# AnneLouisedb/dlwp-benchmark

Measured on AMD Instinct MI355X. Metric: rollout cell-steps/s, higher is better.
Workload: dtype f32 (f16x3: products from two-part f16 splits, 22-bit operands, fp32 accumulate)

## Files before the change

### dlwp_benchmark_amd/csrc/fno_device.hpp

```cpp
#pragma once

#include "common.hpp"

namespace dlwp {
namespace fno {

constexpr int kC = 32;
constexpr int kTrStride = 68;

struct ChanSeg {
  const float* ptr;
  long long bstride;
  int nchan;
  int pad;
};
struct ChanTable {
  ChanSeg seg[4];
};

__device__ __forceinline__ const float* chan_ptr(const ChanTable& t, int c, int b, int HW) {
  const float* p = nullptr;
  int base = 0;
#pragma unroll
  for (int i = 0; i < 4; ++i) {
    const int n = t.seg[i].nchan;
    if (c >= base && c < base + n)
      p = t.seg[i].ptr + (long long)b * t.seg[i].bstride + (long long)(c - base) * HW;
    base += n;
  }
  return p;
}

__device__ __forceinline__ void wave_lds_fence() {
  __builtin_amdgcn_fence(__ATOMIC_ACQ_REL, "wavefront");
  __builtin_amdgcn_wave_barrier();
}

template <int NT, int KP>
__device__ __forceinline__ void fwd_dft_accumulate(const float* s_tr, const float* __restrict__ tt,
                                                   int w0, int lane, f32x4 (&yacc)[NT][KP / 16]) {
  const int j = lane & 15, g = lane >> 4;
#pragma unroll
  for (int s = 0; s < 16; ++s) {
    float bt[KP / 16];
#pragma unroll
    for (int kt = 0; kt < KP / 16; ++kt) bt[kt] = tt[(long long)(w0 + 4 * s + g) * KP + kt * 16 + j];
#pragma unroll
    for (int ct = 0; ct < NT; ++ct) {
      const float a = s_tr[(16 * ct + j) * kTrStride + 4 * s + g];
#pragma unroll
      for (int kt = 0; kt < KP / 16; ++kt) yacc[ct][kt] = mfma16x16x4(a, bt[kt], yacc[ct][kt]);
    }
  }
}

template <int NT, int KP>
__device__ __forceinline__ void store_y(float* __restrict__ ybuf, long long row, int nchan, int lane,
                                        const f32x4 (&yacc)[NT][KP / 16], int c0 = 0) {
  const int j = lane & 15, g = lane >> 4;
#pragma unroll
  for (int ct = 0; ct < NT; ++ct)
#pragma unroll
    for (int kt = 0; kt < KP / 16; ++kt)
      *reinterpret_cast<f32x4*>(ybuf + (row * KP + kt * 16 + j) * nchan + c0 + 16 * ct + 4 * g) = yacc[ct][kt];
}

struct MlpParams {
  ChanTable x;
  int hid;
  int cout;
  const float* w1p;
  const float* b1;
  const float* w2p;
  const float* b2;
  float* out;
  long long out_bstride;
  const float* resid;
  long long resid_bstride;
  float* ybuf;
  const float* tt;
  int B, H, W;
};

template <int CIN_STEPS, bool F16 = false>
__device__ __forceinline__ void lift_segment(const f32x4 (&xs)[CIN_STEPS], const float* s_w1, const float* s_b1,
                                             const u32x4* s_w2, int npair, int lane, const f32x4 (&bias2)[2],
                                             f32x4 (&acc2)[2][4], int ns = CIN_STEPS, bool cin1 = false, float f16_up = 1.f,
                                             float f16_down = 1.f) {
  const int g = lane >> 4;
  f32x4 xbc = {0.f, 0.f, 0.f, 0.f};
  if (cin1) {
#pragma unroll
    for (int q = 0; q < 4; ++q) {
      float v = xs[0][q];
      v += __shfl_xor(v, 16);
      v += __shfl_xor(v, 32);
      xbc[q] = v;
    }
  }
#pragma unroll
  for (int ot = 0; ot < 2; ++ot)
#pragma unroll
    for (int q = 0; q < 4; ++q) acc2[ot][q] = F16 ? bias2[ot] * f16_up : bias2[ot];

  u32x4 bg0[2][3], bg1[2][3];
  f32x4 a1[2][2];
  u32x4 wa[2][3];
  const int nunit = npair * 2;
  auto unit_valu_fc1 = [&](int u, auto qpc) {
    constexpr int qp = decltype(qpc)::value;
#pragma unroll
    for (int tt = 0; tt < 2; ++tt) {
      const int t = 2 * u + tt;
      const f32x4 bb = *reinterpret_cast<const f32x4*>(s_b1 + 16 * t + 4 * g);
      if (cin1) {
        const f32x4 wv = *reinterpret_cast<const f32x4*>(s_w1 + t * 64 + 4 * g);
#pragma unroll
        for (int qq = 0; qq < 2; ++qq)
#pragma unroll
          for (int r = 0; r < 4; ++r) a1[tt][qq][r] = __builtin_fmaf(wv[r], xbc[2 * qp + qq], bb[r]);
        continue;
      }
#pragma unroll
      for (int qq = 0; qq < 2; ++qq) a1[tt][qq] = bb;
#pragma unroll
      for (int s = 0; s < CIN_STEPS; ++s) {
        if (s >= ns) break;
        const float a = s_w1[(t * ns + s) * 64 + lane];
#pragma unroll
        for (int qq = 0; qq < 2; ++qq) a1[tt][qq] = mfma16x16x4(a, xs[s][2 * qp + qq], a1[tt][qq]);
      }
    }
  };
  auto unit_split = [&](u32x4(&bg)[2][3]) {
#pragma unroll
    for (int qq = 0; qq < 2; ++qq)
#pragma unroll
      for (int i = 0; i < 4; ++i) {
        unsigned hh, mm, ll;
        split_pair_x<F16>(a1[i / 2][qq][2 * (i % 2)], a1[i / 2][qq][2 * (i % 2) + 1], hh, mm, ll);
        bg[qq][0][i] = hh;
        bg[qq][1][i] = mm;
        bg[qq][2][i] = ll;
      }
  };
  auto load_wa = [&](int u) {
#pragma unroll
    for (int ot = 0; ot < 2; ++ot)
#pragma unroll
      for (int pp = 0; pp < 3; ++pp) wa[ot][pp] = s_w2[((u * 3 + pp) * 2 + ot) * 64 + lane];
  };
  auto unit_mfma = [&](const u32x4(&bg)[2][3], auto qpc, auto slotc) {
    constexpr int qp = decltype(qpc)::value, slot = decltype(slotc)::value;
    if constexpr (F16) {
      constexpr int PA[3] = {1, 0, 2}, PB[3] = {0, 1, 0};
#pragma unroll
      for (int ot = 0; ot < 2; ++ot)
#pragma unroll
        for (int qq = 0; qq < 2; ++qq)
          acc2[ot][2 * qp + qq] = mfma16x16x32_f16(wa[ot][PA[slot]], bg[qq][PB[slot]], acc2[ot][2 * qp + qq]);
    } else {
    constexpr int PA[6] = {2, 0, 1, 1, 0, 0}, PB[6] = {0, 2, 1, 0, 1, 0};
#pragma unroll
    for (int term = 2 * slot; term < 2 * slot + 2; ++term)
#pragma unroll
      for (int ot = 0; ot < 2; ++ot)
#pragma unroll
        for (int qq = 0; qq < 2; ++qq)
          acc2[ot][2 * qp + qq] = mfma16x16x32_bf16(wa[ot][PA[term]], bg[qq][PB[term]], acc2[ot][2 * qp + qq]);
    }
  };
  using I0 = std::integral_constant<int, 0>;
  using I1 = std::integral_constant<int, 1>;
  using I2 = std::integral_constant<int, 2>;
  auto trip = [&](int u_m, int u_v, const u32x4(&bgm)[2][3], u32x4(&bgv)[2][3], auto qm, auto qv) {
    load_wa(u_m);
    unit_valu_fc1(u_v, qv);
    unit_mfma(bgm, qm, I0{});
    gelu_erf8(a1[0][0], a1[0][1]);
    __builtin_amdgcn_sched_barrier(0);
    unit_mfma(bgm, qm, I1{});
    gelu_erf8(a1[1][0], a1[1][1]);
    __builtin_amdgcn_sched_barrier(0);
    unit_mfma(bgm, qm, I2{});
    unit_split(bgv);
    __builtin_amdgcn_sched_barrier(0);
  };
  unit_valu_fc1(0, I0{});
  gelu_erf8(a1[0][0], a1[0][1]);
  gelu_erf8(a1[1][0], a1[1][1]);
  unit_split(bg0);
  for (int u = 0; u < npair; ++u) {
    trip(u, u, bg0, bg1, I0{}, I1{});
    if (u + 1 < npair) trip(u, u + 1, bg1, bg0, I1{}, I0{});
  }
  load_wa(npair - 1);
  unit_mfma(bg1, I1{}, I0{});
  unit_mfma(bg1, I1{}, I1{});
  unit_mfma(bg1, I1{}, I2{});
  (void)nunit;
  if constexpr (F16) {
#pragma unroll
    for (int ot = 0; ot < 2; ++ot)
#pragma unroll
      for (int q = 0; q < 4; ++q) acc2[ot][q] *= f16_down;
  }

}

constexpr int kLiftTabRange = 32, kLiftTabLog2 = 4;
constexpr int kLiftTabCoefs = 6;
constexpr int kLiftTabStride = kLiftTabCoefs * kC;

__host__ __device__ __forceinline__ int lift_tab_locate(float x, int n_side, float scale, float& v) {
  const float a = fabsf(x) * scale;
  const float fl = floorf(a);
  v = a - fl;
  int k = (int)fl;
  k = k < 0 ? 0 : (k > n_side - 1 ? n_side - 1 : k);
  return x < 0.f ? n_side - 1 - k : n_side + k;
}

__device__ __forceinline__ void lift_from_table(const float* __restrict__ tab, const f32x4& xbc, int g, f32x4 (&vv)[2][4]) {
#pragma unroll
  for (int qp = 0; qp < 2; ++qp) {
    f32x4 c[2][kLiftTabCoefs][2];
    float v[2];
#pragma unroll
    for (int qq = 0; qq < 2; ++qq) {
      const int idx = lift_tab_locate(xbc[2 * qp + qq], kLiftTabRange << kLiftTabLog2, (float)(1 << kLiftTabLog2), v[qq]);
      const f32x4* src = reinterpret_cast<const f32x4*>(tab + (size_t)idx * kLiftTabStride + 4 * g);
#pragma unroll
      for (int k = kLiftTabCoefs - 1; k >= 0; --k) {
        c[qq][k][0] = src[k * (kC / 4)];
        c[qq][k][1] = src[k * (kC / 4) + 4];
      }
    }
#pragma unroll
    for (int qq = 0; qq < 2; ++qq)
#pragma unroll
      for (int ot = 0; ot < 2; ++ot) {
        f32x4 acc = c[qq][kLiftTabCoefs - 1][ot];
#pragma unroll
        for (int k = kLiftTabCoefs - 2; k >= 0; --k)
#pragma unroll
          for (int r = 0; r < 4; ++r) acc[r] = __builtin_fmaf(acc[r], v[qq], c[qq][k][ot][r]);
#pragma unroll
        for (int r = 0; r < 4; ++r) vv[ot][r][2 * qp + qq] = acc[r];
      }
  }
}

template <int CO, bool F16 = false>
__device__ __forceinline__ void proj_segment(const u32x4 (&bx)[4][3], const u32x4* s_w1, const float* s_b1,
                                             const float* s_w2, int ntile, int lane, float (&po)[CO][4], float f16_down = 1.f) {
  const int g = lane >> 4;
#pragma unroll
  for (int co = 0; co < CO; ++co)
#pragma unroll
    for (int q = 0; q < 4; ++q) po[co][q] = 0.f;
  auto fc1 = [&](int t, f32x4(&a1)[4]) {
    const f32x4 bb = *reinterpret_cast<const f32x4*>(s_b1 + 16 * t + 4 * g);
    u32x4 wa[3];
#pragma unroll
    for (int pp = 0; pp < 3; ++pp) wa[pp] = s_w1[(t * 3 + pp) * 64 + lane];
#pragma unroll
    for (int q = 0; q < 4; ++q) a1[q] = mfma_x<F16>(wa, bx[q], bb);
  };
  f32x4 a_cur[4], a_nxt[4], g_prev[4], g_new[4];
  fc1(0, a_cur);
  fc1(ntile > 1 ? 1 : 0, a_nxt);
#pragma unroll
  for (int q = 0; q < 4; ++q) g_prev[q] = F16 ? a_cur[q] * f16_down : a_cur[q];
  gelu_erf8(g_prev[0], g_prev[1]);
  gelu_erf8(g_prev[2], g_prev[3]);
#pragma unroll
  for (int q = 0; q < 4; ++q) a_cur[q] = a_nxt[q];
  u32x4 wa[3], wa_n[3];
  f32x4 w2v[CO], w2v_n[CO], bb, bb_n;
  {
    const int tn = ntile > 2 ? 2 : ntile - 1;
#pragma unroll
    for (int pp = 0; pp < 3; ++pp) wa[pp] = s_w1[(tn * 3 + pp) * 64 + lane];
#pragma unroll
    for (int co = 0; co < CO; ++co) w2v[co] = *reinterpret_cast<const f32x4*>(s_w2 + co * 16 + 4 * g);
    bb = *reinterpret_cast<const f32x4*>(s_b1 + 16 * tn + 4 * g);
  }
  for (int t = 1; t < ntile; ++t) {
    {
      const int tn2 = (t + 2 < ntile) ? t + 2 : ntile - 1;
#pragma unroll
      for (int pp = 0; pp < 3; ++pp) wa_n[pp] = s_w1[(tn2 * 3 + pp) * 64 + lane];
#pragma unroll
      for (int co = 0; co < CO; ++co) w2v_n[co] = *reinterpret_cast<const f32x4*>(s_w2 + (t * CO + co) * 16 + 4 * g);
      bb_n = *reinterpret_cast<const f32x4*>(s_b1 + 16 * tn2 + 4 * g);
    }
#pragma unroll
    for (int i = 0; i < 2; ++i) {
      a_nxt[2 * i] = mfma_x<F16>(wa, bx[2 * i], bb);
      a_nxt[2 * i + 1] = mfma_x<F16>(wa, bx[2 * i + 1], bb);
      g_new[2 * i] = F16 ? a_cur[2 * i] * f16_down : a_cur[2 * i];
      g_new[2 * i + 1] = F16 ? a_cur[2 * i + 1] * f16_down : a_cur[2 * i + 1];
      gelu_erf8(g_new[2 * i], g_new[2 * i + 1]);
#pragma unroll
      for (int co = 0; co < CO; ++co)
#pragma unroll
        for (int qq = 2 * i; qq < 2 * i + 2; ++qq)
#pragma unroll
          for (int r = 0; r < 4; ++r) po[co][qq] = fmaf(w2v[co][r], g_prev[qq][r], po[co][qq]);
      __builtin_amdgcn_sched_barrier(0);
    }
#pragma unroll
    for (int q = 0; q < 4; ++q) {
      g_prev[q] = g_new[q];
      a_cur[q] = a_nxt[q];
    }
#pragma unroll
    for (int pp = 0; pp < 3; ++pp) wa[pp] = wa_n[pp];
#pragma unroll
    for (int co = 0; co < CO; ++co) w2v[co] = w2v_n[co];
    bb = bb_n;
  }
  {
    const int t = ntile - 1;
#pragma unroll
    for (int co = 0; co < CO; ++co) {
      const f32x4 w2 = *reinterpret_cast<const f32x4*>(s_w2 + (t * CO + co) * 16 + 4 * g);
#pragma unroll
      for (int q = 0; q < 4; ++q)
#pragma unroll
        for (int r = 0; r < 4; ++r) po[co][q] = fmaf(w2[r], g_prev[q][r], po[co][q]);
    }
  }
}

struct LayerParams {
  const float* x;
  float* y;
  const float* wsp;
  const u32x4* wsb;
  const float* bias;
  const float* zbuf;
  const float* t;
  const float* tt;
  float* ybuf;
  int B, H, W;
  int stagger;
};

__device__ __forceinline__ float2 cfma(float2 a, float2 b, float2 c) {
  return float2{fmaf(a.x, b.x, fmaf(-a.y, b.y, c.x)), fmaf(a.x, b.y, fmaf(a.y, b.x, c.y))};
}

constexpr int kTrunkF16Shift = 3;
constexpr float kTrunkF16Up = 16384.0f, kTrunkF16Down = 1.0f / 16384.0f;

}
}
```

Baseline: 2.363 billion.

## Restructure projection pipeline into half-tile stages with register-light prefetch

Rewrites the projection segment's software pipeline so MFMA for the next tile, GELU for the current half-tile, and the FC2 FMAs for the previous half-tile are interleaved at half-tile granularity. The separate next-iteration copies of weights and activations are dropped in favour of single buffers reloaded in place, which lowers register pressure. Inline asm register pins keep each accumulator chain grouped. The added scheduling barriers fix the instruction order, but reloading buffers in place could expose LDS latency.

```diff
diff --git a/dlwp_benchmark_amd/csrc/fno_device.hpp b/dlwp_benchmark_amd/csrc/fno_device.hpp
--- a/dlwp_benchmark_amd/csrc/fno_device.hpp
+++ b/dlwp_benchmark_amd/csrc/fno_device.hpp
@@ -255,83 +255,68 @@
 __device__ __forceinline__ void proj_segment(const u32x4 (&bx)[4][3], const u32x4* s_w1, const float* s_b1,
                                              const float* s_w2, int ntile, int lane, float (&po)[CO][4], float f16_down = 1.f) {
   const int g = lane >> 4;
+  u32x4 wa[3];
+  f32x4 bb, w2v[CO];
+  auto load_l1 = [&](int t) {
+#pragma unroll
+    for (int pp = 0; pp < 3; ++pp) wa[pp] = s_w1[(t * 3 + pp) * 64 + lane];
+    bb = *reinterpret_cast<const f32x4*>(s_b1 + 16 * t + 4 * g);
+  };
+  auto load_l2 = [&](int t) {
+#pragma unroll
+    for (int co = 0; co < CO; ++co) w2v[co] = *reinterpret_cast<const f32x4*>(s_w2 + (t * CO + co) * 16 + 4 * g);
+  };
+  auto down = [&](const f32x4& a) -> f32x4 { return F16 ? a * f16_down : a; };
 #pragma unroll
   for (int co = 0; co < CO; ++co)
 #pragma unroll
     for (int q = 0; q < 4; ++q) po[co][q] = 0.f;
-  auto fc1 = [&](int t, f32x4(&a1)[4]) {
-    const f32x4 bb = *reinterpret_cast<const f32x4*>(s_b1 + 16 * t + 4 * g);
-    u32x4 wa[3];
-#pragma unroll
-    for (int pp = 0; pp < 3; ++pp) wa[pp] = s_w1[(t * 3 + pp) * 64 + lane];
-#pragma unroll
-    for (int q = 0; q < 4; ++q) a1[q] = mfma_x<F16>(wa, bx[q], bb);
-  };
-  f32x4 a_cur[4], a_nxt[4], g_prev[4], g_new[4];
-  fc1(0, a_cur);
-  fc1(ntile > 1 ? 1 : 0, a_nxt);
-#pragma unroll
-  for (int q = 0; q < 4; ++q) g_prev[q] = F16 ? a_cur[q] * f16_down : a_cur[q];
-  gelu_erf8(g_prev[0], g_prev[1]);
-  gelu_erf8(g_prev[2], g_prev[3]);
-#pragma unroll
-  for (int q = 0; q < 4; ++q) a_cur[q] = a_nxt[q];
-  u32x4 wa[3], wa_n[3];
-  f32x4 w2v[CO], w2v_n[CO], bb, bb_n;
-  {
-    const int tn = ntile > 2 ? 2 : ntile - 1;
-#pragma unroll
-    for (int pp = 0; pp < 3; ++pp) wa[pp] = s_w1[(tn * 3 + pp) * 64 + lane];
-#pragma unroll
-    for (int co = 0; co < CO; ++co) w2v[co] = *reinterpret_cast<const f32x4*>(s_w2 + co * 16 + 4 * g);
-    bb = *reinterpret_cast<const f32x4*>(s_b1 + 16 * tn + 4 * g);
-  }
+  auto fma2 = [&](int q0, const f32x4(&gg)[2]) {
+#pragma unroll
+    for (int co = 0; co < CO; ++co)
+#pragma unroll
+      for (int qq = 0; qq < 2; ++qq) {
+        float acc = po[co][q0 + qq];
+        asm("" : "+v"(acc));
+#pragma unroll
+        for (int r = 0; r < 4; ++r) acc = fmaf(w2v[co][r], gg[qq][r], acc);
+        asm("" : "+v"(acc));
+        po[co][q0 + qq] = acc;
+      }
+  };
+  f32x4 a[4], ga[2], gb[2];
+  load_l1(0);
+#pragma unroll
+  for (int q = 0; q < 4; ++q) a[q] = mfma_x<F16>(wa, bx[q], bb);
+  load_l1(ntile > 1 ? 1 : 0);
+  load_l2(0);
+  ga[0] = down(a[0]); ga[1] = down(a[1]);
+  gb[0] = down(a[2]); gb[1] = down(a[3]);
+#pragma unroll
+  for (int q = 0; q < 4; ++q) a[q] = mfma_x<F16>(wa, bx[q], bb);
+  load_l1(ntile > 2 ? 2 : ntile - 1);
+  gelu_erf8(ga[0], ga[1]);
+  gelu_erf8(gb[0], gb[1]);
+  fma2(0, ga);
   for (int t = 1; t < ntile; ++t) {
-    {
-      const int tn2 = (t + 2 < ntile) ? t + 2 : ntile - 1;
-#pragma unroll
-      for (int pp = 0; pp < 3; ++pp) wa_n[pp] = s_w1[(tn2 * 3 + pp) * 64 + lane];
-#pragma unroll
-      for (int co = 0; co < CO; ++co) w2v_n[co] = *reinterpret_cast<const f32x4*>(s_w2 + (t * CO + co) * 16 + 4 * g);
-      bb_n = *reinterpret_cast<const f32x4*>(s_b1 + 16 * tn2 + 4 * g);
-    }
-#pragma unroll
-    for (int i = 0; i < 2; ++i) {
-      a_nxt[2 * i] = mfma_x<F16>(wa, bx[2 * i], bb);
-      a_nxt[2 * i + 1] = mfma_x<F16>(wa, bx[2 * i + 1], bb);
-      g_new[2 * i] = F16 ? a_cur[2 * i] * f16_down : a_cur[2 * i];
-      g_new[2 * i + 1] = F16 ? a_cur[2 * i + 1] * f16_down : a_cur[2 * i + 1];
-      gelu_erf8(g_new[2 * i], g_new[2 * i + 1]);
-#pragma unroll
-      for (int co = 0; co < CO; ++co)
-#pragma unroll
-        for (int qq = 2 * i; qq < 2 * i + 2; ++qq)
-#pragma unroll
-          for (int r = 0; r < 4; ++r) po[co][qq] = fmaf(w2v[co][r], g_prev[qq][r], po[co][qq]);
-      __builtin_amdgcn_sched_barrier(0);
-    }
-#pragma unroll
-    for (int q = 0; q < 4; ++q) {
-      g_prev[q] = g_new[q];
-      a_cur[q] = a_nxt[q];
-    }
-#pragma unroll
-    for (int pp = 0; pp < 3; ++pp) wa[pp] = wa_n[pp];
-#pragma unroll
-    for (int co = 0; co < CO; ++co) w2v[co] = w2v_n[co];
-    bb = bb_n;
-  }
-  {
-    const int t = ntile - 1;
-#pragma unroll
-    for (int co = 0; co < CO; ++co) {
-      const f32x4 w2 = *reinterpret_cast<const f32x4*>(s_w2 + (t * CO + co) * 16 + 4 * g);
-#pragma unroll
-      for (int q = 0; q < 4; ++q)
-#pragma unroll
-        for (int r = 0; r < 4; ++r) po[co][q] = fmaf(w2[r], g_prev[q][r], po[co][q]);
-    }
-  }
+    ga[0] = down(a[0]); ga[1] = down(a[1]);
+    __builtin_amdgcn_sched_barrier(0);
+    a[0] = mfma_x<F16>(wa, bx[0], bb);
+    a[1] = mfma_x<F16>(wa, bx[1], bb);
+    gelu_erf8(ga[0], ga[1]);
+    fma2(2, gb);
+    load_l2(t);
+    __builtin_amdgcn_sched_barrier(0);
+    gb[0] = down(a[2]); gb[1] = down(a[3]);
+    __builtin_amdgcn_sched_barrier(0);
+    a[2] = mfma_x<F16>(wa, bx[2], bb);
+    a[3] = mfma_x<F16>(wa, bx[3], bb);
+    load_l1(t + 2 < ntile ? t + 2 : ntile - 1);
+    gelu_erf8(gb[0], gb[1]);
+    fma2(0, ga);
+    __builtin_amdgcn_sched_barrier(0);
+  }
+  fma2(2, gb);
 }
 
 struct LayerParams {
```

Result: faster. 2.429 billion, median of 6 (+2.8%).
